# LIS-TU-Berlin/SVN-ICP

Measured on AMD Instinct MI355X. Metric: scan-pair registrations/sec at N particles x M source pts, 1/2/4/8 GPU, higher is better.
Workload: dtype f64; 1 GPU; C3: 128 particles SVN-ICP, 131072-pt source vs 262144-pt target, K=100, I=20, max_dist=1.0, lr=1.0, SVNFullGrad=False, correspondence=fast, early stop off; synthetic 64-beam scans (seed 20250718); particles=128, target_points=262144, knn_count=100, parallelism=single GPU

## Files before the change

svn-icp_amd/csrc/stein_split_device.hpp:

```cpp
#pragma once
#include <cstdlib>
#include "kernels.hpp"
#include "stein_common.hpp"
#include "search_limits.hpp"

namespace svnicp {

namespace {

typedef float v4f __attribute__((ext_vector_type(4)));
#define SVNICP_CONST_AS __attribute__((address_space(4)))

__device__ __forceinline__ float pack_slot(float v, unsigned int mask, unsigned int bits) {
  return __uint_as_float((__float_as_uint(v) & ~mask) | bits);
}
__device__ __forceinline__ float imin_f(float a, float b) {
  const int x = (int)__float_as_uint(a), y = (int)__float_as_uint(b);
  return __uint_as_float((unsigned int)(x < y ? x : y));
}
__device__ __forceinline__ float imax_f(float a, float b) {
  const int x = (int)__float_as_uint(a), y = (int)__float_as_uint(b);
  return __uint_as_float((unsigned int)(x > y ? x : y));
}

typedef __bf16 bf2 __attribute__((ext_vector_type(2)));
typedef float f2v __attribute__((ext_vector_type(2)));
typedef __bf16 bf8 __attribute__((ext_vector_type(8)));
typedef unsigned int u4v __attribute__((ext_vector_type(4)));

__device__ __forceinline__ unsigned int cvt_pk_bf16(float lo, float hi) {
  const f2v v = {lo, hi};
  return __builtin_bit_cast(unsigned int, __builtin_convertvector(v, bf2));
}
__device__ __forceinline__ bf8 split_a3(float x) {
  const unsigned int r0 = cvt_pk_bf16(x, x);
  const float e1 = x - __uint_as_float(r0 & 0xffff0000u);
  const unsigned int r1 = cvt_pk_bf16(x, e1);
  const float e2 = e1 - __uint_as_float(r1 & 0xffff0000u);
  const unsigned int r2 = cvt_pk_bf16(e1, e2);
  const u4v t = {r0, r1, r2, r2};
  return __builtin_bit_cast(bf8, t);
}
__device__ __forceinline__ bf8 split_b3(float x) {
  const float e1 = x - __uint_as_float(cvt_pk_bf16(0.0f, x));
  const float e2 = e1 - __uint_as_float(cvt_pk_bf16(0.0f, e1));
  const unsigned int q0 = cvt_pk_bf16(x, e1);
  const unsigned int q1 = cvt_pk_bf16(e2, x);
  const unsigned int q2 = cvt_pk_bf16(e1, x);
  const u4v t = {q0, q1, q2, 0u};
  return __builtin_bit_cast(bf8, t);
}
__device__ __forceinline__ float pack_slot3(float v, unsigned int bits) {
  return __uint_as_float(__builtin_amdgcn_bitop3_b32(__float_as_uint(v), 31u, bits, 0xBA));
}
__device__ __forceinline__ float fmin_raw(float a, float b) { return __builtin_elementwise_minimum(a, b); }
__device__ __forceinline__ float fmax_raw(float a, float b) { return __builtin_elementwise_maximum(a, b); }
__device__ __forceinline__ float fmed3_raw(float a, float b, float c) { return __builtin_amdgcn_fmed3f(a, b, c); }
__device__ __forceinline__ float fmin3_raw(float a, float b, float c) { return __builtin_elementwise_minimum(__builtin_elementwise_minimum(a, b), c); }
constexpr int kQueueCap = 1024;

template <int G>
__device__ __forceinline__ int exact_nearest_of_k(const AccumArgs& a, const double (*pose)[64], int64_t b, int pl, int K, int sub) {
  constexpr int NIT = 128 / G;
  const double* sp = a.src + 3 * b;
  const int32_t* ci = a.cand + (size_t)b * K;
  int64_t ti[NIT];
#pragma unroll
  for (int i = 0; i < NIT; ++i) {
    const int k = sub + i * G;
    int64_t t = ci[k < K ? k : 0];
    ti[i] = t < 0 ? 0 : (t >= a.M ? a.M - 1 : t);
  }
  double rx[NIT], ry[NIT], rz[NIT];
#pragma unroll
  for (int i = 0; i < NIT; ++i) {
    const double* r = a.tgt + 3 * ti[i];
    rx[i] = r[0]; ry[i] = r[1]; rz[i] = r[2];
  }
  const double u0 = sp[0], u1 = sp[1], u2 = sp[2];
  const double t0 = (u0 * pose[0][pl] + u1 * pose[1][pl] + u2 * pose[2][pl]) + pose[9][pl];
  const double t1 = (u0 * pose[3][pl] + u1 * pose[4][pl] + u2 * pose[5][pl]) + pose[10][pl];
  const double t2 = (u0 * pose[6][pl] + u1 * pose[7][pl] + u2 * pose[8][pl]) + pose[11][pl];
  double bd = __builtin_huge_val(), d_first = 0.0;
  int bk = 0x7fffffff;
#pragma unroll
  for (int i = 0; i < NIT; ++i) {
    const int k = sub + i * G;
    const double dx = t0 - rx[i], dy = t1 - ry[i], dz = t2 - rz[i];
    const double d = (dx * dx + dy * dy) + dz * dz;
    if (k == 0) d_first = d;
    if (k < K && (d < bd || (d == bd && k < bk))) { bd = d; bk = k; }
  }
#pragma unroll
  for (int off = G / 2; off > 0; off >>= 1) {
    const double od = __shfl_xor(bd, off, kWave);
    const int ok = __shfl_xor(bk, off, kWave);
    if (od < bd || (od == bd && ok < bk)) { bd = od; bk = ok; }
  }
  const double d0 = __shfl(d_first, (threadIdx.x & (kWave - 1)) & ~(G - 1), kWave);
  return (d0 != d0 || bk == 0x7fffffff) ? 0 : bk;
}

#ifndef SVNICP_SEARCH_EPS_U
#define SVNICP_SEARCH_EPS_U 54
#endif
constexpr float kEpsBf16 = (float)SVNICP_SEARCH_EPS_U * 5.9604644775390625e-08f;

#ifndef SVNICP_SEARCH_WAVES
#define SVNICP_SEARCH_WAVES 4
#endif
template <int PW, int WP, int NRB, bool TAIL>
__device__ __forceinline__ void search_body(const AccumArgs& a, int bx, int by) {
  if (a.ctl[0]) return;
  if (a.fin_iteration >= 0 && bx == 0 && by == 0) {
    __shared__ double sh_fin[NT];
    __shared__ int sh_fin_stop;
    const int ftid = threadIdx.x, FP = a.fin_P;
    double fs = 0.0;
    for (int p = ftid; p < FP; p += NT) fs += a.fin_norms[p];
    sh_fin[ftid] = fs;
    __syncthreads();
    for (int off = NT / 2; off > 0; off >>= 1) {
      if (ftid < off) sh_fin[ftid] += sh_fin[ftid + off];
      __syncthreads();
    }
    if (ftid == 0) {
      const double m = sh_fin[0] / FP;
      const int stop = (float)m < (float)a.fin_thr;
      if (stop) { a.fin_ctl[0] = 1; a.fin_ctl[1] = a.fin_iteration + 1; }
      sh_fin_stop = stop;
    }
    __syncthreads();
    if (sh_fin_stop) return;
    for (int e = ftid; e < 6 * FP; e += NT) a.fin_history[(size_t)a.fin_iteration * 6 * FP + e] = (float)a.fin_pose[e];
  }
  constexpr int BW = kWave / PW;
  constexpr int CBP = PW / 16;
  constexpr int NPT = 4 / CBP;
  constexpr int ST = 4 * BW;
  constexpr bool PIPE = NPT == 1;
  constexpr int NTILE = 4 * NRB + (TAIL ? 1 : 0);
  constexpr int RS = 16 * (((4 * NTILE + 15) / 16) | 1);
  __shared__ float4 s_rows[4][NPT][4][RS / 4];
  __shared__ float4 s_scr4[4][64];
  __shared__ double s_pose[WP][12][64];
  __shared__ unsigned int s_queue[kQueueCap];
  __shared__ unsigned int s_qn, s_qsteps;
  const int tid = threadIdx.x;
  if (tid == 0) { s_qn = 0u; s_qsteps = 0u; }
#pragma unroll
  for (int i = 0; i < kQueueCap / NT; ++i) s_queue[tid + i * NT] = 0xffffffffu;
  const int lane = tid & (kWave - 1);
  const int wave = __builtin_amdgcn_readfirstlane(tid >> 6);
  const int pl = lane % PW, bs = lane / PW;
  const int mj = lane & 15, mk = lane >> 4;
  const int pbase = by * (WP * PW);
  for (int g = wave; g < WP; g += 4) {
    const int p = a.p_lo + pbase + g * PW + pl;
    const double* rp = a.Rtot + 12 * (size_t)(p < a.p_hi ? p : a.p_lo);
#pragma unroll
    for (int i = 0; i < 12; ++i) s_pose[g][i][lane] = rp[i];
  }
  const int K = a.K;
  const SVNICP_CONST_AS v4f* ctab = (const SVNICP_CONST_AS v4f*)a.tablea;
  float* const rows_w = reinterpret_cast<float*>(&s_rows[wave][0][mk][0]) + mj;
  const int64_t blk_lo = (int64_t)bx * a.spts_per_block;
  const int64_t blk_hi = (blk_lo + a.spts_per_block < a.B) ? blk_lo + a.spts_per_block : a.B;
  static_assert(BW <= kSearchPointsPerStep, "search_limits.hpp bounds the pair offsets for at most this many points per step");
  __syncthreads();
  const int64_t nfirst = blk_lo + wave * BW;

  int pend_idx = 0;
  int32_t* pend_row = a.kidx;
  unsigned int pend_off4 = 0;
  bool pend_have = false;
  v4f alo_n, ahi_n;
  double sa_n = 0.0;
  float c_n = 0.0f;
  auto fetch_point = [&](int64_t nn) {
    const double* base = lane < 3 ? a.src + 3 * nn : a.anchor + 3 * nn - 3;
    sa_n = base[lane < 6 ? lane : 3];
    c_n = a.cmax[nn];
  };
  v4f ralo_n[PIPE ? 1 : NPT], rahi_n[PIPE ? 1 : NPT];
  auto fetch_rows = [&](int64_t n0, int pt) {
    int64_t bq = n0 + pt;
    bq = bq < blk_hi ? bq : (n0 < blk_hi ? n0 : blk_lo);
    const SVNICP_CONST_AS v4f* rowp = ctab + (size_t)bq * 128 + lane;
    ralo_n[pt] = rowp[0];
    rahi_n[pt] = ralo_n[pt];
    if constexpr (NRB > 4) rahi_n[pt] = rowp[64];
  };
  if constexpr (!PIPE) {
#pragma unroll
    for (int pt = 0; pt < NPT; ++pt) fetch_rows(nfirst, pt);
  }
  if constexpr (PIPE) {
    fetch_point(nfirst < blk_hi ? nfirst : blk_lo);
    const SVNICP_CONST_AS v4f* rowp = ctab + (size_t)(nfirst < blk_hi ? nfirst : blk_lo) * 128 + lane;
    alo_n = rowp[0];
    ahi_n = alo_n;
    if constexpr (NRB > 4) ahi_n = rowp[64];
  }

  for (int64_t n = nfirst; n < blk_hi; n += ST) {
    const int64_t b = n + bs;
    const bool inb = b < blk_hi;
    double s0, s1, s2, a0, a1, a2;
    float C;
    if constexpr (PIPE) {
      s0 = rdlane_f64(sa_n, 0); s1 = rdlane_f64(sa_n, 1); s2 = rdlane_f64(sa_n, 2);
      a0 = rdlane_f64(sa_n, 3); a1 = rdlane_f64(sa_n, 4); a2 = rdlane_f64(sa_n, 5);
      C = __uint_as_float((unsigned int)__builtin_amdgcn_readfirstlane((int)__float_as_uint(c_n)));
    } else {
      const int64_t bl = inb ? b : n;
      const double* sp = a.src + 3 * bl;
      const double* an = a.anchor + 3 * bl;
      s0 = sp[0]; s1 = sp[1]; s2 = sp[2];
      a0 = an[0]; a1 = an[1]; a2 = an[2];
      C = a.cmax[bl];
    }

    bf8 afr[NRB];
    auto split_rows = [&](v4f alo, v4f ahi, int pt) {
#pragma unroll
      for (int rb = 0; rb < NRB; ++rb) {
        const float v = rb == 0 ? alo.x : rb == 1 ? alo.y : rb == 2 ? alo.z : rb == 3 ? alo.w
                      : rb == 4 ? ahi.x : rb == 5 ? ahi.y : rb == 6 ? ahi.z : ahi.w;
        afr[rb] = split_a3(v);
        rows_w[pt * 4 * RS + 16 * rb] = v;
      }
      if constexpr (TAIL) {
        const float v = NRB == 4 ? ahi.x : NRB == 5 ? ahi.y : NRB == 6 ? ahi.z : ahi.w;
        if (mj < 4) rows_w[pt * 4 * RS + 16 * NRB] = v;
      }
    };
    if constexpr (PIPE) {
      const v4f alo = alo_n, ahi = ahi_n;
      int64_t nn = n + ST;
      nn = nn < blk_hi ? nn : n;
      const SVNICP_CONST_AS v4f* rowp = ctab + (size_t)nn * 128 + lane;
      alo_n = rowp[0];
      if constexpr (NRB > 4) ahi_n = rowp[64];
      fetch_point(nn);
      __builtin_amdgcn_wave_barrier();
      split_rows(alo, ahi, 0);
    }

#pragma nounroll
    for (int g = 0; g < WP; ++g) {
      float E, mm0, mm1, mm2;
      {
        const double (*pose)[64] = s_pose[g];
        const double T0 = (s0 * pose[0][lane] + s1 * pose[1][lane] + s2 * pose[2][lane]) + pose[9][lane];
        const double T1 = (s0 * pose[3][lane] + s1 * pose[4][lane] + s2 * pose[5][lane]) + pose[10][lane];
        const double T2 = (s0 * pose[6][lane] + s1 * pose[7][lane] + s2 * pose[8][lane]) + pose[11][lane];
        const float xf0 = (float)(T0 - a0), xf1 = (float)(T1 - a1), xf2 = (float)(T2 - a2);
        const float X2 = __builtin_amdgcn_sqrtf(__builtin_fmaf(xf0, xf0, __builtin_fmaf(xf1, xf1, xf2 * xf2))) * 1.000002f;
        const float Cq = __builtin_fmaf(5.9604644775390625e-08f, X2, C);
        E = kEpsBf16 * Cq * __builtin_fmaf(2.0f, X2, Cq);
        mm0 = -2.0f * xf0; mm1 = -2.0f * xf1; mm2 = -2.0f * xf2;
        if (g > 0) __builtin_amdgcn_wave_barrier();
        s_scr4[wave][lane] = make_float4(mm0, mm1, mm2, 1.0f);
        __builtin_amdgcn_wave_barrier();
      }
      const float* scr4f = reinterpret_cast<const float*>(s_scr4[wave]);
      float b1[4], b2[4];
      float braw[4];
#pragma unroll
      for (int cb = 0; cb < 4; ++cb) braw[cb] = scr4f[(16 * cb + mj) * 4 + mk];

#pragma unroll
      for (int cb = 0; cb < 4; ++cb) {
        if constexpr (!PIPE) {
          if (cb % CBP == 0) {
            split_rows(ralo_n[cb / CBP], rahi_n[cb / CBP], cb / CBP);
            fetch_rows(n + ST, cb / CBP);
          }
        }
        const bf8 bfr = split_b3(braw[cb]);
        const v4f zero = {0.0f, 0.0f, 0.0f, 0.0f};
        float m1 = 0.0f, m2 = 0.0f, wp = 0.0f, rp = 0.0f, pend0 = 0.0f, pend1 = 0.0f;
        int np = 0;
        bool have_m = false;
        bool have_p = false;
        v4f dcur = __builtin_amdgcn_mfma_f32_16x16x32_bf16(afr[0], bfr, zero, 0, 0, 0);
        v4f dnext = dcur;
        if (NRB > 1) dnext = __builtin_amdgcn_mfma_f32_16x16x32_bf16(afr[NRB > 1 ? 1 : 0], bfr, zero, 0, 0, 0);
#pragma unroll
        for (int rb = 0; rb < NRB; ++rb) {
          v4f dn2 = dnext;
          if (rb + 2 < NRB) dn2 = __builtin_amdgcn_mfma_f32_16x16x32_bf16(afr[rb + 2 < NRB ? rb + 2 : 0], bfr, zero, 0, 0, 0);
          const float pk = pack_slot3(fmin_raw(fmin3_raw(dcur[0], dcur[1], dcur[2]), dcur[3]), 4u * rb);
          if (np == 0) { pend0 = pk; np = 1; }
          else if (np == 1) { pend1 = pk; np = 2; }
          else {
            np = 0;
            const float w = fmin3_raw(pend0, pend1, pk), r = fmed3_raw(pend0, pend1, pk);
            if (!have_p) { wp = w; rp = r; have_p = true; }
            else {
              have_p = false;
              if (!have_m) {
                m1 = fmin_raw(wp, w);
                m2 = fmin3_raw(fmax_raw(wp, w), rp, r);
                have_m = true;
              } else {
                const float md = fmed3_raw(m1, wp, w);
                m2 = fmin_raw(fmin3_raw(m2, rp, r), md);
                m1 = fmin3_raw(m1, wp, w);
              }
            }
          }
          dcur = dnext; dnext = dn2;
        }
        if (!have_m) { m1 = __builtin_huge_valf(); m2 = __builtin_huge_valf(); }
        if (have_p) { const float t = fmax_raw(m1, wp); m1 = fmin_raw(m1, wp); m2 = fmin3_raw(t, m2, rp); }
        if (np >= 1) { m2 = fmed3_raw(m1, m2, pend0); m1 = fmin_raw(m1, pend0); }
        if (np >= 2) { m2 = fmed3_raw(m1, m2, pend1); m1 = fmin_raw(m1, pend1); }
        b1[cb] = m1; b2[cb] = m2;
      }
#pragma unroll
      for (int cb = 0; cb < 4; ++cb) b1[cb] = __uint_as_float(__builtin_amdgcn_bitop3_b32(__float_as_uint(b1[cb]), 3u, (unsigned int)mk, 0xBA));
      auto merge2 = [&](float p1, float q1, float p2, float q2, float& o1, float& o2) {
        o1 = fmin_raw(p1, q1);
        o2 = fmin_raw(fmax_raw(p1, q1), fmin_raw(p2, q2));
      };
      float b1own, b2own;
      {
        float h1[2], h2[2];
#pragma unroll
        for (int j = 0; j < 2; ++j) {
          const auto r1 = __builtin_amdgcn_permlane16_swap(__float_as_uint(b1[2 * j]), __float_as_uint(b1[2 * j + 1]), false, false);
          const auto r2 = __builtin_amdgcn_permlane16_swap(__float_as_uint(b2[2 * j]), __float_as_uint(b2[2 * j + 1]), false, false);
          merge2(__uint_as_float(r1[0]), __uint_as_float(r1[1]), __uint_as_float(r2[0]), __uint_as_float(r2[1]), h1[j], h2[j]);
        }
        const auto r1 = __builtin_amdgcn_permlane32_swap(__float_as_uint(h1[0]), __float_as_uint(h1[1]), false, false);
        const auto r2 = __builtin_amdgcn_permlane32_swap(__float_as_uint(h2[0]), __float_as_uint(h2[1]), false, false);
        merge2(__uint_as_float(r1[0]), __uint_as_float(r1[1]), __uint_as_float(r2[0]), __uint_as_float(r2[1]), b1own, b2own);
      }
      auto score_tile = [&](int tile, float* sc) {
        const float4 cx = s_rows[wave][bs][0][tile], cy = s_rows[wave][bs][1][tile];
        const float4 cz = s_rows[wave][bs][2][tile], cc = s_rows[wave][bs][3][tile];
        sc[0] = __builtin_fmaf(cx.x, mm0, __builtin_fmaf(cy.x, mm1, __builtin_fmaf(cz.x, mm2, cc.x)));
        sc[1] = __builtin_fmaf(cx.y, mm0, __builtin_fmaf(cy.y, mm1, __builtin_fmaf(cz.y, mm2, cc.y)));
        sc[2] = __builtin_fmaf(cx.z, mm0, __builtin_fmaf(cy.z, mm1, __builtin_fmaf(cz.z, mm2, cc.z)));
        sc[3] = __builtin_fmaf(cx.w, mm0, __builtin_fmaf(cy.w, mm1, __builtin_fmaf(cz.w, mm2, cc.w)));
      };
      if constexpr (TAIL) {
        float sc[4];
        score_tile(4 * NRB, sc);
        const float pk = pack_slot3(fmin_raw(fmin3_raw(sc[0], sc[1], sc[2]), sc[3]), 4u * NRB);
        b2own = fmed3_raw(b1own, b2own, pk);
        b1own = fmin_raw(b1own, pk);
      }

      const int pin = g * PW + pl;
      const bool valid = inb && (a.p_lo + pbase + pin) < a.p_hi;
      int tile = (int)(__float_as_uint(b1own) & 31u);
      tile = tile < NTILE ? tile : NTILE - 1;
      const float thr = 2.0f * E + 3.83e-06f * (__builtin_fabsf(b1own) + __builtin_fabsf(b2own)) + 1.0e-30f;
      const bool tiles_ok = b2own - b1own > thr;
      float pk4[4];
      {
        if constexpr (!PIPE) __builtin_amdgcn_wave_barrier();
        float sc[4];
        score_tile(tile, sc);
#pragma unroll
        for (int t = 0; t < 4; ++t) pk4[t] = __uint_as_float(__builtin_amdgcn_bitop3_b32(__float_as_uint(sc[t]), 3u, (unsigned int)t, 0xBA));
      }
      const float w3 = fmin3_raw(pk4[0], pk4[1], pk4[2]), r3 = fmed3_raw(pk4[0], pk4[1], pk4[2]);
      const float v1 = fmin_raw(w3, pk4[3]), v2 = fmed3_raw(w3, r3, pk4[3]);
      const float thrv = 2.0f * E + 4.76837158203125e-07f * (__builtin_fabsf(v1) + __builtin_fabsf(v2)) + 1.0e-30f;
      int kb = 4 * tile + (int)(__float_as_uint(v1) & 3u);
      const bool ambiguous = valid & (!tiles_ok | !(v2 - v1 > thrv) | (kb >= K));
      kb = kb < K ? kb : K - 1;
      unsigned long long am = __ballot(ambiguous);
      if (am) {
        const int cnt = __builtin_popcountll(am);
        int base = 0;
        if (lane == 0) { base = (int)atomicAdd(&s_qn, (unsigned int)cnt); atomicAdd(&s_qsteps, 1u); }
        base = __builtin_amdgcn_readfirstlane(base);
        if (base + cnt <= kQueueCap) {
          if (ambiguous) {
            const int rank = __builtin_popcountll(am & ((1ull << lane) - 1ull));
            s_queue[base + rank] = ((unsigned int)(b - blk_lo) << 8) | (unsigned int)pin;
          }
        } else {
          do {
            const int L = (int)__builtin_ctzll(am);
            am &= am - 1;
            const int ke = exact_nearest_of_k<kWave>(a, s_pose[g], n + L / PW, L % PW, K, lane);
            if (lane == L) kb = ke;
          } while (am);
        }
      }
      if (pend_have) *(int32_t*)((char*)pend_row + pend_off4) = pend_idx;
      pend_have = inb;
      pend_row = a.kidx + n * a.Ppad + pbase;
      if (inb) {
        const unsigned int bl = (unsigned int)bs;
        const unsigned int off = bl * (unsigned int)a.Ppad + (unsigned int)pin;
        (a.kbest + n * a.Ppad + pbase)[off] = (uint8_t)kb;
        pend_off4 = 4u * off;
        pend_idx = *(const int32_t*)((const char*)(a.cand + n * K) + 4u * (bl * (unsigned int)K + (unsigned int)kb));
      }
    }
    __builtin_amdgcn_wave_barrier();
  }

  if (pend_have) *(int32_t*)((char*)pend_row + pend_off4) = pend_idx;
  __syncthreads();
  {
    const unsigned int total = s_qn < (unsigned int)kQueueCap ? s_qn : (unsigned int)kQueueCap;
    constexpr int kExactLanes = 32;
    const int sub = lane & (kExactLanes - 1);
    for (unsigned int e = (unsigned int)(tid / kExactLanes); e < total; e += NT / kExactLanes) {
      const unsigned int ent = s_queue[e];
      if (ent == 0xffffffffu) continue;
      const int64_t be = blk_lo + (int64_t)(ent >> 8);
      const int pin = (int)(ent & 0xffu);
      const int ke = exact_nearest_of_k<kExactLanes>(a, s_pose[pin / PW], be, pin % PW, K, sub);
      if (sub == 0) {
        a.kbest[(size_t)be * a.Ppad + (pbase + pin)] = (uint8_t)ke;
        a.kidx[(size_t)be * a.Ppad + (pbase + pin)] = a.cand[(size_t)be * K + ke];
      }
    }
    if (tid == 0 && a.ambig_count && s_qsteps) { atomicAdd(a.ambig_count, (int)s_qsteps); atomicAdd(a.ambig_count + 1, (int)s_qn); }
  }
}

template <int PW, int WP, int NRB, bool TAIL>
__global__ __launch_bounds__(NT, (PW == 16 || WP == 4) ? 3 : SVNICP_SEARCH_WAVES) void k_stein_search_bf16(AccumArgs a) {
  search_body<PW, WP, NRB, TAIL>(a, xcd_block((int)blockIdx.x, (int)gridDim.x), (int)blockIdx.y);
}

template <int PW, int WP, bool PLAIN, bool SVGD = false>
__device__ __forceinline__ void accumulate_body(const AccumArgs& a, int bx, int by, double* lds) {
  if (a.ctl[0]) return;
  constexpr int BW = kWave / PW;
  constexpr int WB = 4 / WP;
#ifndef SVNICP_ACCUM_U
#define SVNICP_ACCUM_U 4
#endif
  constexpr int U = SVNICP_ACCUM_U;
  const int tid = threadIdx.x;
  const int lane = tid & (kWave - 1);
  const int wave = __builtin_amdgcn_readfirstlane(tid >> 6);
  const int wp = wave % WP, wb = wave / WP;
  const int pl = lane % PW, bs = lane / PW;
  const int pidx = by * (WP * PW) + wp * PW + pl;
  const int p = a.p_lo + pidx;
  const bool pvalid = p < a.p_hi;

  double Rt[9], tt[3];
  {
    const double* rp = a.Rtot + 12 * (size_t)(pvalid ? p : a.p_lo);
#pragma unroll
    for (int i = 0; i < 9; ++i) Rt[i] = rp[i];
#pragma unroll
    for (int i = 0; i < 3; ++i) tt[i] = rp[9 + i];
  }
  double acc[kNSums];
#pragma unroll
  for (int i = 0; i < kNSums; ++i) acc[i] = 0.0;
  const int K = a.K;
  const int64_t blk_lo = (int64_t)bx * a.pts_per_block;
  const int64_t blk_hi = (blk_lo + a.pts_per_block < a.B) ? blk_lo + a.pts_per_block : a.B;
  constexpr int STEP = WB * BW;
  const SVNICP_CONST_AS double* csrc = (const SVNICP_CONST_AS double*)a.src;
  const SVNICP_CONST_AS int32_t* ccand = (const SVNICP_CONST_AS int32_t*)a.cand;
  const SVNICP_CONST_AS double* ctgt = (const SVNICP_CONST_AS double*)a.tgt;
  const uint8_t* kbp = a.kbest + pidx;
  const int32_t* kip = a.kidx + pidx;

  const int32_t* fullp = (!PLAIN && a.full_idx) ? a.full_idx + (size_t)(pvalid ? p : a.p_lo) * a.B : nullptr;
  auto load_kb = [&](int64_t n) -> int {
    const int64_t b = n + bs;
    const int64_t bc = b < blk_hi ? b : blk_lo;
    if (PLAIN) return kip[(size_t)bc * a.Ppad];
    if (fullp) return fullp[bc];
    return (int)kbp[(size_t)bc * a.Ppad];
  };
  const double c3d = 3.0 / a.max_dist;
  auto accumulate = [&](double on, double s0, double s1, double s2, double q0, double q1, double q2) {
    const double T0 = (s0 * Rt[0] + s1 * Rt[1] + s2 * Rt[2]) + tt[0];
    const double T1 = (s0 * Rt[3] + s1 * Rt[4] + s2 * Rt[5]) + tt[1];
    const double T2 = (s0 * Rt[6] + s1 * Rt[7] + s2 * Rt[8]) + tt[2];
    const double dx = T0 - q0, dy = T1 - q1, dz = T2 - q2;
    const double best = (dx * dx + dy * dy) + dz * dz;
    const bool in = best < a.max_dist;
    const double mf = in ? on : 0.0;
    const double x = in ? mf * best : 0.0;
    const double r0 = __builtin_amdgcn_rsq(x + 0x1p-1000);
    const double sa = x * r0, h0 = 0.5 * r0;
    const double ea = fma(-h0, sa, 0.5);
    const double sb = fma(sa, ea, sa);
    const double nn = fma(fma(-sb, sb, x), h0, sb);
    const double den = fma(c3d, nn, 1.0);
    const double y0 = __builtin_amdgcn_rcp(den);
    const double y1 = fma(y0, fma(-den, y0, 1.0), y0);
    const double wq = fma(y1, fma(-den, y1, 1.0), y1);
    const double w = on * (wq * wq);
    const double we = mf * w;
    const double e0 = we * dx, e1 = we * dy, e2 = we * dz;
    const double w0 = we * s0, w1 = we * s1, w2 = we * s2;
    acc[0] += w;
    acc[1] += w0; acc[2] += w1; acc[3] += w2;
    if (PLAIN ? SVGD : (a.svgd != 0)) acc[4] += (((T0 + T1) + T2) != 0.0) ? mf : 0.0;
    else acc[4] = fma(w0, s0, acc[4]);
    acc[5] = fma(w0, s1, acc[5]); acc[6] = fma(w0, s2, acc[6]);
    acc[7] = fma(w1, s1, acc[7]); acc[8] = fma(w1, s2, acc[8]); acc[9] = fma(w2, s2, acc[9]);
    acc[10] += e0; acc[11] += e1; acc[12] += e2;
    acc[13] = fma(e0, s0, acc[13]); acc[14] = fma(e0, s1, acc[14]); acc[15] = fma(e0, s2, acc[15]);
    acc[16] = fma(e1, s0, acc[16]); acc[17] = fma(e1, s1, acc[17]); acc[18] = fma(e1, s2, acc[18]);
    acc[19] = fma(e2, s0, acc[19]); acc[20] = fma(e2, s1, acc[20]); acc[21] = fma(e2, s2, acc[21]);
  };

  const int64_t n0 = blk_lo + wb * BW;
  int kbn[U];
#pragma unroll
  for (int u = 0; u < U; ++u) kbn[u] = load_kb(n0 + u * STEP);
  for (int64_t n = n0; n < blk_hi; n += U * STEP) {
    int kb[U];
    int64_t ti[U];
#pragma unroll
    for (int u = 0; u < U; ++u) {
      kb[u] = kbn[u];
      const int64_t b = n + u * STEP + bs;
      const int64_t bl = b < blk_hi ? b : blk_lo;
      const int64_t t = (PLAIN || fullp) ? (int64_t)kb[u] : (int64_t)ccand[(size_t)bl * K + kb[u]];
      ti[u] = t < 0 ? 0 : (t >= a.M ? a.M - 1 : t);
    }
#pragma unroll
    for (int u = 0; u < U; ++u) kbn[u] = load_kb(n + (U + u) * STEP);
    double q[U][3];
#pragma unroll
    for (int u = 0; u < U; ++u) {
      const SVNICP_CONST_AS double* r = ctgt + 3 * ti[u];
      q[u][0] = r[0]; q[u][1] = r[1]; q[u][2] = r[2];
    }
#pragma unroll
    for (int u = 0; u < U; ++u) {
      const int64_t b = n + u * STEP + bs;
      const bool valid = pvalid && b < blk_hi;
      const int64_t bl = b < blk_hi ? b : blk_lo;
      const SVNICP_CONST_AS double* sp = csrc + 3 * bl;
      const double s0 = sp[0], s1 = sp[1], s2 = sp[2];
      if (!PLAIN && a.corr && valid) a.corr[(size_t)p * a.B + b] = kb[u];
      accumulate(b < blk_hi ? 1.0 : 0.0, s0, s1, s2, q[u][0], q[u][1], q[u][2]);
    }
  }
  {
    const double t = (acc[10] + acc[11]) + acc[12];
    if (t != t) {
#pragma unroll
      for (int i = 0; i < kNSums; ++i) acc[i] = t;
    }
  }

#pragma unroll
  for (int off = PW; off < kWave; off <<= 1) {
#pragma unroll
    for (int i = 0; i < kNSums; ++i) acc[i] += __shfl_xor(acc[i], off, kWave);
  }
  if constexpr (WB > 1) {
    double* red = lds;
    if (wb > 0 && bs == 0) {
      double* r = red + ((size_t)(wb - 1) * (WP * PW) + wp * PW + pl) * kNSums;
#pragma unroll
      for (int i = 0; i < kNSums; ++i) r[i] = acc[i];
    }
    __syncthreads();
    if (wb == 0 && bs == 0) {
      for (int o = 0; o < WB - 1; ++o) {
        const double* r = red + ((size_t)o * (WP * PW) + wp * PW + pl) * kNSums;
#pragma unroll
        for (int i = 0; i < kNSums; ++i) acc[i] += r[i];
      }
    }
  }
  if (wb == 0 && bs == 0) {
    double* out = a.partial + ((size_t)bx * a.Ppad + pidx) * kNSums;
#pragma unroll
    for (int i = 0; i < kNSums; ++i) out[i] = acc[i];
  }
}

template <int PW, int WP, bool PLAIN, bool SVGD = false>
__global__ __launch_bounds__(NT, (PLAIN && SVGD) ? 4 : 3) void k_stein_accumulate_w(AccumArgs a) {
  extern __shared__ __align__(16) double lds[];
  accumulate_body<PW, WP, PLAIN, SVGD>(a, xcd_block((int)blockIdx.x, (int)gridDim.x), (int)blockIdx.y, lds);
}

}
}
```

Baseline: 145.5 registrations/s.

## Compute search query vectors in float relative to a block reference pose

In the pipelined search path, each block picks a reference pose (first particle) and a reference source point, then precomputes per-particle pose deltas and per-point offsets in float with rigorous error bounds. The per-particle-per-point transform in the inner loop drops its f64 matrix-vector product and becomes a few float FMAs, and the epsilon for the ambiguity test is widened to cover the relative-frame rounding. Point data is now fetched once per 64 steps as a lane-distributed batch and read back with readlane, replacing a per-step fetch. Shared-memory f64 poses are replaced by float relative data, and exact fallbacks read poses from global memory. The wider epsilon may send more entries to the exact queue.

Result: no change. 146.9 registrations/s, median of 6 (+1.0%).

```diff
diff --git a/svn-icp_amd/csrc/search_relative.hpp b/svn-icp_amd/csrc/search_relative.hpp
--- /dev/null
+++ b/svn-icp_amd/csrc/search_relative.hpp
@@ -0,0 +1,93 @@
+#pragma once
+#include <cstdint>
+
+#if defined(__HIPCC__) || defined(__CUDACC__)
+#define SVNICP_REL_FN __host__ __device__ inline
+#else
+#define SVNICP_REL_FN inline
+#endif
+
+namespace svnicp {
+
+constexpr int kRelParticleFloats = 14;
+constexpr int kRelPointFloats = 8;
+constexpr float kRelFloor = 0x1p-90f;
+constexpr float kRelUp = 1.00001f;
+
+struct RelRef {
+  double R[9], t[3];
+  double s0[3];
+  double rcol, t1, s01;
+};
+
+SVNICP_REL_FN double rel_abs(double x) { return __builtin_fabs(x); }
+SVNICP_REL_FN float rel_absf(float x) { return __builtin_fabsf(x); }
+SVNICP_REL_FN float rel_floor(float x) { return x < kRelFloor ? kRelFloor : x; }
+
+SVNICP_REL_FN void rel_ref_norms(RelRef& r) {
+  double c = 0.0;
+#pragma unroll
+  for (int j = 0; j < 3; ++j) {
+    const double cj = (rel_abs(r.R[j]) + rel_abs(r.R[3 + j])) + rel_abs(r.R[6 + j]);
+    c = cj > c ? cj : c;
+  }
+  r.rcol = c * 1.000001;
+  r.t1 = ((rel_abs(r.t[0]) + rel_abs(r.t[1])) + rel_abs(r.t[2])) * 1.000001;
+  r.s01 = ((rel_abs(r.s0[0]) + rel_abs(r.s0[1])) + rel_abs(r.s0[2])) * 1.000001;
+}
+
+SVNICP_REL_FN void rel_particle(const double* pose, const RelRef& r, float* o) {
+  double dt1 = 0.0;
+#pragma unroll
+  for (int i = 0; i < 3; ++i) {
+    const double d0 = pose[3 * i] - r.R[3 * i], d1 = pose[3 * i + 1] - r.R[3 * i + 1], d2 = pose[3 * i + 2] - r.R[3 * i + 2];
+    const double dt = pose[9 + i] - r.t[i];
+    const double dtp = __builtin_fma(d2, r.s0[2], __builtin_fma(d1, r.s0[1], __builtin_fma(d0, r.s0[0], dt)));
+    o[3 * i] = (float)(-2.0 * d0); o[3 * i + 1] = (float)(-2.0 * d1); o[3 * i + 2] = (float)(-2.0 * d2);
+    o[9 + i] = (float)(-2.0 * dtp);
+    dt1 += rel_abs(dt);
+  }
+  const float N = (rel_absf(o[9]) + rel_absf(o[10])) + rel_absf(o[11]);
+  o[12] = rel_floor(kRelUp * (4.0f * N + (float)(0x1p-24 * dt1)));
+  float rho = 0.0f;
+  bool bad = false;
+#pragma unroll
+  for (int j = 0; j < 3; ++j) {
+    const float cj = (rel_absf(o[j]) + rel_absf(o[3 + j])) + rel_absf(o[6 + j]);
+    bad = bad | !(cj == cj);
+    rho = cj > rho ? cj : rho;
+  }
+  o[13] = bad ? __builtin_nanf("") : rel_floor(kRelUp * rho);
+}
+
+SVNICP_REL_FN void rel_point(const double* s, const double* an, const RelRef& r, float* o) {
+#pragma unroll
+  for (int i = 0; i < 3; ++i) {
+    const double T = (s[0] * r.R[3 * i] + s[1] * r.R[3 * i + 1] + s[2] * r.R[3 * i + 2]) + r.t[i];
+    o[i] = (float)(-2.0 * (T - an[i]));
+    o[3 + i] = (float)(s[i] - r.s0[i]);
+  }
+  const double s1 = (rel_abs(s[0]) + rel_abs(s[1])) + rel_abs(s[2]);
+  const float U = (rel_absf(o[0]) + rel_absf(o[1])) + rel_absf(o[2]);
+  const float S = (rel_absf(o[3]) + rel_absf(o[4])) + rel_absf(o[5]);
+  o[6] = kRelUp * (U + (float)(0x1p-24 * (r.rcol * s1 + r.t1)));
+  o[7] = rel_floor(kRelUp * (5.0f * S + (float)(0x1p-24 * (s1 + r.s01))));
+}
+
+SVNICP_REL_FN void rel_mm(const float* D, const float* u, const float* sp, float* mm) {
+#pragma unroll
+  for (int i = 0; i < 3; ++i) {
+    const float p = __builtin_fmaf(D[3 * i], sp[0], __builtin_fmaf(D[3 * i + 1], sp[1], __builtin_fmaf(D[3 * i + 2], sp[2], D[9 + i])));
+    mm[i] = p + u[i];
+  }
+}
+SVNICP_REL_FN float rel_delta_u(float Np, float rhop, float Ub, float Sb) { return __builtin_fmaf(rhop, Sb, Np) + Ub; }
+
+SVNICP_REL_FN float search_eps(float C, float X2, float dl, float eps_u) {
+  const float u = 5.9604644775390625e-08f;
+  const float X2p = __builtin_fmaf(dl, 0.5f * u, X2);
+  const float Cq = X2p * u + C;
+  return (eps_u * u * Cq) * __builtin_fmaf(dl, 1.000001f / eps_u, __builtin_fmaf(2.0f, X2p, Cq));
+}
+
+}
diff --git a/svn-icp_amd/csrc/stein_split_device.hpp b/svn-icp_amd/csrc/stein_split_device.hpp
--- a/svn-icp_amd/csrc/stein_split_device.hpp
+++ b/svn-icp_amd/csrc/stein_split_device.hpp
@@ -3,6 +3,7 @@
 #include "kernels.hpp"
 #include "stein_common.hpp"
 #include "search_limits.hpp"
+#include "search_relative.hpp"
 
 namespace svnicp {
 
@@ -60,7 +61,7 @@
 constexpr int kQueueCap = 1024;
 
 template <int G>
-__device__ __forceinline__ int exact_nearest_of_k(const AccumArgs& a, const double (*pose)[64], int64_t b, int pl, int K, int sub) {
+__device__ __forceinline__ int exact_nearest_of_k(const AccumArgs& a, const double* pose, int ps, int64_t b, int K, int sub) {
   constexpr int NIT = 128 / G;
   const double* sp = a.src + 3 * b;
   const int32_t* ci = a.cand + (size_t)b * K;
@@ -78,9 +79,9 @@
     rx[i] = r[0]; ry[i] = r[1]; rz[i] = r[2];
   }
   const double u0 = sp[0], u1 = sp[1], u2 = sp[2];
-  const double t0 = (u0 * pose[0][pl] + u1 * pose[1][pl] + u2 * pose[2][pl]) + pose[9][pl];
-  const double t1 = (u0 * pose[3][pl] + u1 * pose[4][pl] + u2 * pose[5][pl]) + pose[10][pl];
-  const double t2 = (u0 * pose[6][pl] + u1 * pose[7][pl] + u2 * pose[8][pl]) + pose[11][pl];
+  const double t0 = (u0 * pose[0] + u1 * pose[ps] + u2 * pose[2 * ps]) + pose[9 * ps];
+  const double t1 = (u0 * pose[3 * ps] + u1 * pose[4 * ps] + u2 * pose[5 * ps]) + pose[10 * ps];
+  const double t2 = (u0 * pose[6 * ps] + u1 * pose[7 * ps] + u2 * pose[8 * ps]) + pose[11 * ps];
   double bd = __builtin_huge_val(), d_first = 0.0;
   int bk = 0x7fffffff;
 #pragma unroll
@@ -143,7 +144,8 @@
   constexpr int RS = 16 * (((4 * NTILE + 15) / 16) | 1);
   __shared__ float4 s_rows[4][NPT][4][RS / 4];
   __shared__ float4 s_scr4[4][64];
-  __shared__ double s_pose[WP][12][64];
+  __shared__ double s_pose[PIPE ? 1 : WP][12][PIPE ? 1 : 64];
+  __shared__ float s_rel[PIPE ? WP : 1][kRelParticleFloats][PIPE ? 64 : 1];
   __shared__ unsigned int s_queue[kQueueCap];
   __shared__ unsigned int s_qn, s_qsteps;
   const int tid = threadIdx.x;
@@ -155,17 +157,47 @@
   const int pl = lane % PW, bs = lane / PW;
   const int mj = lane & 15, mk = lane >> 4;
   const int pbase = by * (WP * PW);
-  for (int g = wave; g < WP; g += 4) {
-    const int p = a.p_lo + pbase + g * PW + pl;
-    const double* rp = a.Rtot + 12 * (size_t)(p < a.p_hi ? p : a.p_lo);
-#pragma unroll
-    for (int i = 0; i < 12; ++i) s_pose[g][i][lane] = rp[i];
+  const int64_t blk_lo = (int64_t)bx * a.spts_per_block;
+  const int64_t blk_hi = (blk_lo + a.spts_per_block < a.B) ? blk_lo + a.spts_per_block : a.B;
+  RelRef ref;
+  if constexpr (!PIPE) {
+    for (int g = wave; g < WP; g += 4) {
+      const int p = a.p_lo + pbase + g * PW + pl;
+      const double* rp = a.Rtot + 12 * (size_t)(p < a.p_hi ? p : a.p_lo);
+#pragma unroll
+      for (int i = 0; i < 12; ++i) s_pose[g][i][lane] = rp[i];
+    }
+  } else {
+    {
+      const int p = a.p_lo + pbase;
+      const double* rp = a.Rtot + 12 * (size_t)(p < a.p_hi ? p : a.p_lo);
+#pragma unroll
+      for (int i = 0; i < 9; ++i) { const double v = rdlane_f64(rp[i], 0); ref.R[i] = (v - v == 0.0) ? v : 0.0; }
+#pragma unroll
+      for (int i = 0; i < 3; ++i) { const double v = rdlane_f64(rp[9 + i], 0); ref.t[i] = (v - v == 0.0) ? v : 0.0; }
+    }
+    {
+      const SVNICP_CONST_AS double* sp = (const SVNICP_CONST_AS double*)a.src + 3 * (blk_lo < a.B ? blk_lo : 0);
+      const double o0 = sp[0], o1 = sp[1], o2 = sp[2];
+      const bool fin = ((o0 - o0) + (o1 - o1)) + (o2 - o2) == 0.0;
+      ref.s0[0] = fin ? o0 : 0.0; ref.s0[1] = fin ? o1 : 0.0; ref.s0[2] = fin ? o2 : 0.0;
+    }
+    rel_ref_norms(ref);
+    for (int g = wave; g < WP; g += 4) {
+      const int p = a.p_lo + pbase + g * PW + lane;
+      const double* rp = a.Rtot + 12 * (size_t)(p < a.p_hi ? p : a.p_lo);
+      double v[12];
+#pragma unroll
+      for (int i = 0; i < 12; ++i) v[i] = rp[i];
+      float o[kRelParticleFloats];
+      rel_particle(v, ref, o);
+#pragma unroll
+      for (int i = 0; i < kRelParticleFloats; ++i) s_rel[g][i][lane] = o[i];
+    }
   }
   const int K = a.K;
   const SVNICP_CONST_AS v4f* ctab = (const SVNICP_CONST_AS v4f*)a.tablea;
   float* const rows_w = reinterpret_cast<float*>(&s_rows[wave][0][mk][0]) + mj;
-  const int64_t blk_lo = (int64_t)bx * a.spts_per_block;
-  const int64_t blk_hi = (blk_lo + a.spts_per_block < a.B) ? blk_lo + a.spts_per_block : a.B;
   static_assert(BW <= kSearchPointsPerStep, "search_limits.hpp bounds the pair offsets for at most this many points per step");
   __syncthreads();
   const int64_t nfirst = blk_lo + wave * BW;
@@ -175,13 +207,19 @@
   unsigned int pend_off4 = 0;
   bool pend_have = false;
   v4f alo_n, ahi_n;
-  double sa_n = 0.0;
-  float c_n = 0.0f;
-  auto fetch_point = [&](int64_t nn) {
-    const double* base = lane < 3 ? a.src + 3 * nn : a.anchor + 3 * nn - 3;
-    sa_n = base[lane < 6 ? lane : 3];
-    c_n = a.cmax[nn];
+  float pt_rel[kRelPointFloats], pt_c = 0.0f;
+#pragma unroll
+  for (int i = 0; i < kRelPointFloats; ++i) pt_rel[i] = 0.0f;
+  auto fetch_batch = [&](int64_t n0) {
+    int64_t bq = n0 + (int64_t)ST * lane;
+    bq = bq < blk_hi ? bq : n0;
+    const double* sp = a.src + 3 * bq;
+    const double* an = a.anchor + 3 * bq;
+    const double sv[3] = {sp[0], sp[1], sp[2]}, av[3] = {an[0], an[1], an[2]};
+    pt_c = a.cmax[bq];
+    rel_point(sv, av, ref, pt_rel);
   };
+  int bstep = 0;
   v4f ralo_n[PIPE ? 1 : NPT], rahi_n[PIPE ? 1 : NPT];
   auto fetch_rows = [&](int64_t n0, int pt) {
     int64_t bq = n0 + pt;
@@ -196,7 +234,6 @@
     for (int pt = 0; pt < NPT; ++pt) fetch_rows(nfirst, pt);
   }
   if constexpr (PIPE) {
-    fetch_point(nfirst < blk_hi ? nfirst : blk_lo);
     const SVNICP_CONST_AS v4f* rowp = ctab + (size_t)(nfirst < blk_hi ? nfirst : blk_lo) * 128 + lane;
     alo_n = rowp[0];
     ahi_n = alo_n;
@@ -206,12 +243,17 @@
   for (int64_t n = nfirst; n < blk_hi; n += ST) {
     const int64_t b = n + bs;
     const bool inb = b < blk_hi;
-    double s0, s1, s2, a0, a1, a2;
+    double s0 = 0.0, s1 = 0.0, s2 = 0.0, a0 = 0.0, a1 = 0.0, a2 = 0.0;
     float C;
+    float pu[3] = {0.0f, 0.0f, 0.0f}, ps[3] = {0.0f, 0.0f, 0.0f}, pUb = 0.0f, pSb = 0.0f;
     if constexpr (PIPE) {
-      s0 = rdlane_f64(sa_n, 0); s1 = rdlane_f64(sa_n, 1); s2 = rdlane_f64(sa_n, 2);
-      a0 = rdlane_f64(sa_n, 3); a1 = rdlane_f64(sa_n, 4); a2 = rdlane_f64(sa_n, 5);
-      C = __uint_as_float((unsigned int)__builtin_amdgcn_readfirstlane((int)__float_as_uint(c_n)));
+      if (bstep == 0) fetch_batch(n);
+      auto rl = [&](float v) { return __uint_as_float((unsigned int)__builtin_amdgcn_readlane((int)__float_as_uint(v), bstep)); };
+#pragma unroll
+      for (int i = 0; i < 3; ++i) { pu[i] = rl(pt_rel[i]); ps[i] = rl(pt_rel[3 + i]); }
+      pUb = rl(pt_rel[6]); pSb = rl(pt_rel[7]);
+      C = rl(pt_c);
+      bstep = (bstep + 1) & (kWave - 1);
     } else {
       const int64_t bl = inb ? b : n;
       const double* sp = a.src + 3 * bl;
@@ -242,7 +284,6 @@
       const SVNICP_CONST_AS v4f* rowp = ctab + (size_t)nn * 128 + lane;
       alo_n = rowp[0];
       if constexpr (NRB > 4) ahi_n = rowp[64];
-      fetch_point(nn);
       __builtin_amdgcn_wave_barrier();
       split_rows(alo, ahi, 0);
     }
@@ -250,7 +291,20 @@
 #pragma nounroll
     for (int g = 0; g < WP; ++g) {
       float E, mm0, mm1, mm2;
-      {
+      if constexpr (PIPE) {
+        float D[12], mm[3];
+#pragma unroll
+        for (int i = 0; i < 12; ++i) D[i] = s_rel[g][i][lane];
+        rel_mm(D, pu, ps, mm);
+        asm("" : "+v"(mm[1]));
+        const float dl = rel_delta_u(s_rel[g][12][lane], s_rel[g][13][lane], pUb, pSb);
+        mm0 = mm[0]; mm1 = mm[1]; mm2 = mm[2];
+        const float X2 = __builtin_amdgcn_sqrtf(__builtin_fmaf(mm0, mm0, __builtin_fmaf(mm1, mm1, mm2 * mm2))) * 0.500001f;
+        E = search_eps(C, X2, dl, (float)SVNICP_SEARCH_EPS_U);
+        if (g > 0) __builtin_amdgcn_wave_barrier();
+        s_scr4[wave][lane] = make_float4(mm0, mm1, mm2, 1.0f);
+        __builtin_amdgcn_wave_barrier();
+      } else {
         const double (*pose)[64] = s_pose[g];
         const double T0 = (s0 * pose[0][lane] + s1 * pose[1][lane] + s2 * pose[2][lane]) + pose[9][lane];
         const double T1 = (s0 * pose[3][lane] + s1 * pose[4][lane] + s2 * pose[5][lane]) + pose[10][lane];
@@ -389,7 +443,9 @@
           do {
             const int L = (int)__builtin_ctzll(am);
             am &= am - 1;
-            const int ke = exact_nearest_of_k<kWave>(a, s_pose[g], n + L / PW, L % PW, K, lane);
+            int ke;
+            if constexpr (PIPE) ke = exact_nearest_of_k<kWave>(a, a.Rtot + 12 * (size_t)(a.p_lo + pbase + g * PW + L), 1, n, K, lane);
+            else ke = exact_nearest_of_k<kWave>(a, &s_pose[g][0][L % PW], 64, n + L / PW, K, lane);
             if (lane == L) kb = ke;
           } while (am);
         }
@@ -419,7 +475,9 @@
       if (ent == 0xffffffffu) continue;
       const int64_t be = blk_lo + (int64_t)(ent >> 8);
       const int pin = (int)(ent & 0xffu);
-      const int ke = exact_nearest_of_k<kExactLanes>(a, s_pose[pin / PW], be, pin % PW, K, sub);
+      int ke;
+      if constexpr (PIPE) ke = exact_nearest_of_k<kExactLanes>(a, a.Rtot + 12 * (size_t)(a.p_lo + pbase + pin), 1, be, K, sub);
+      else ke = exact_nearest_of_k<kExactLanes>(a, &s_pose[pin / PW][0][pin % PW], 64, be, K, sub);
       if (sub == 0) {
         a.kbest[(size_t)be * a.Ppad + (pbase + pin)] = (uint8_t)ke;
         a.kidx[(size_t)be * a.Ppad + (pbase + pin)] = a.cand[(size_t)be * K + ke];
```
